# taldatech/soft-intro-vae-pytorch

Measured on AMD Instinct MI355X. Metric: training images/sec (whole node) at 256x256 bs128, higher is better.
Workload: dtype f32; 1 GPU; soft_intro_vae celeb256 256x256 zdim=512 channels=[64, 128, 256, 512, 512, 512], full E-step + D-step iteration; global_batch=128, per_gpu_batch=128, parallelism=dp1, decoder_forward_reuse=True, hip_graph=False, batchnorm=local

## Files before the change

### soft-intro-vae-pytorch_amd/csrc/conv_wino4_kernel.inc

```
template <bool PRO>
__global__ void __launch_bounds__(W4_NT, 1) W4_KERNEL_NAME(Wino4Args a) {
  constexpr int CK = W4_CK, RS = W4_RS, PLANE = W4_PLANE, XBUF = W4_XBUF, VBUF = W4_VBUF;
  __shared__ __attribute__((aligned(16))) float raw0[XBUF];
  __shared__ __attribute__((aligned(16))) float raw1[XBUF];
  __shared__ __attribute__((aligned(16))) float vx[VBUF + W4_EXF];
#define RAWB(BUF) ((BUF) ? raw1 : raw0)
  __shared__ float4 pro4[PRO ? W4_PRO_MAX : 1];

  const int tid = threadIdx.x, lane = tid & 63;
  const int wave = __builtin_amdgcn_readfirstlane(tid >> 6);
  const int l31 = lane & 31, hh = lane >> 5;
  const int wj = wave % 6, ws = wave / 6;
  const int H = a.H, W = a.W, HW = H * W;
  const int tx = l31 & 7, ty = l31 >> 3;

  const int tp = wave >> 2;
  const int ti = (wave & 3) * 64 + lane, tt = ti & 31, tc = ti >> 5;
  const int trb = tc * PLANE + 4 * (tt >> 3) * RS + 4 * (tt & 7) + 4;
  const int jA = tp == 0 ? 1 : (tp == 1 ? 3 : 0), jB = tp == 0 ? 2 : (tp == 1 ? 4 : 5);
  const int tvb = tc * 32 + tt;
  const float t_al = tp == 0 ? -4.f : -1.f;
  const float t_be = tp == 0 ? 1.f : 2.f;
  const float t_ga = tp == 0 ? -4.f : -2.f;
  const bool pair05 = tp == 2;
#if W4_GRID
  const unsigned long long seam_m0 = a.seam_c0, seam_m5 = a.seam_c5, seam_mr0 = a.seam_r0, seam_mr5 = a.seam_r5;
  const int two_w = W4_PXW, two_h = W4_PXH, two_mask = a.W - 1, two_hmask = a.H - 1, two_img = a.Ci * a.H * a.W;
  const int two_nx = W4_PXW >> a.iw_l2, two_ipi = two_nx * (W4_PXH >> a.ih_l2);
#else
  const unsigned long long seam_m0 = 0x1010101010101010ull, seam_m5 = 0x0808080808080808ull;
  const int two_w = a.two ? 32 : a.W, two_mask = a.two ? 15 : -1, two_img = a.two ? a.Ci * a.H * a.W : 0;
#endif
  const int vrb = (wj * CK + hh) * 32 + l31;

  const int dsub = wave % 3, dpl0 = wave / 3;
  const int pg = dsub * 64 + lane, prow = pg / 10, pk = pg - prow * 10;
  const bool pvalid = pg < 180;

  const int n_items = a.n_items;
  const int nchunks = a.cps;
  const int ksteps = nchunks * (CK / 2);
  const __amdgpu_buffer_rsrc_t ursrc = make_rsrc(a.up, 36ull * a.Ci_pad * a.Co_pad * 4ull);
  const unsigned va0 = (unsigned)(hh * a.Co_pad + ws * 32 + l31) * 24u;
  const unsigned ua_step = (unsigned)a.Co_pad * 24u;

  int item = blockIdx.x;
  if (a.xcd_group) item = ((int)blockIdx.x & 7) * ((int)gridDim.x >> 3) + ((int)blockIdx.x >> 3);
  int b, r0, c0, co0, pt;
  int cbase = 0, kslice = 0;
  __amdgpu_buffer_rsrc_t xrsrc;
  unsigned xo, ua_base;
  int pseg = 0;
#if W4_GRID
#define W4_SETUP_IMG                                                     \
    b = two_ipi * pt;                                                    \
    xrsrc = make_rsrc(a.x + (size_t)b * a.Ci * HW, (unsigned long long)two_ipi * a.Ci * HW * 4ull); \
    const int r = r0 - 1 + prow, c = c0 - 4 + 4 * pk;                    \
    xo = (pvalid && r >= 0 && r < two_h && c >= 0 && c < two_w)          \
             ? (unsigned)(((r >> a.ih_l2) * two_nx + (c >> a.iw_l2)) * two_img + (r & two_hmask) * W + (c & two_mask)) * 4u \
             : SIVAE_OOB;
#else
#define W4_SETUP_IMG                                                     \
    b = a.two ? 2 * pt : b;                                              \
    xrsrc = make_rsrc(a.x + (size_t)b * a.Ci * HW, (unsigned long long)(a.two ? 2 : 1) * a.Ci * HW * 4ull); \
    const int r = r0 - 1 + prow, c = c0 - 4 + 4 * pk;                    \
    xo = (pvalid && r >= 0 && r < H && c >= 0 && c < two_w)              \
             ? (unsigned)((c >> 4) * two_img + r * W + (c & two_mask)) * 4u : SIVAE_OOB;
#endif
#define W4_SETUP(ITEM)                                                   \
  {                                                                      \
    const int co_tile = (ITEM) % a.n_co_tiles;                           \
    const int iq_ = (ITEM) / a.n_co_tiles;                               \
    kslice = iq_ % a.ksl;                                                \
    pt = iq_ / a.ksl;                                                    \
    cbase = kslice * a.cps * CK;                                         \
    const int tbx = pt % a.nbw;                                          \
    const int t2 = pt / a.nbw;                                           \
    const int tby = t2 % a.nbh;                                          \
    b = t2 / a.nbh;                                                      \
    r0 = tby * W4_PXH;                                                   \
    c0 = tbx * W4_PXW;                                                   \
    co0 = co_tile * W4_TCO;                                              \
    W4_SETUP_IMG                                                         \
    ua_base = (unsigned)((wj * a.Ci_pad + cbase) * a.Co_pad + co0) * 24u; \
    if (PRO) pseg = (b / a.pro_seg_images) * a.Ci_pad + cbase;           \
  }
#define W4_DMA1(CH, BUF, N)                                              \
  if (!((W4_ABLATE & 1) && item >= 0)) {                                 \
    const int ck = dpl0 + 4 * (N);                                       \
    const int ci = cbase + (CH)*CK + ck;                                 \
    const int cic = ci < a.Ci ? ci : a.Ci - 1;                           \
    __builtin_amdgcn_raw_ptr_buffer_load_lds(                            \
        xrsrc, (float __attribute__((address_space(3)))*)(RAWB(BUF) + ck * PLANE + dsub * 256), 16, xo, \
        (unsigned)cic * (unsigned)HW * 4u, 0, 0);                        \
  }
#define W4_FIXUP(CH, BUF, XO, PSEG)                                      \
  {                                                                      \
    const float msk_ = (XO) != SIVAE_OOB ? 1.f : 0.f;                    \
    _Pragma("unroll") for (int n_ = 0; n_ < 2; ++n_) {                   \
      const int ck = dpl0 + 4 * n_;                                      \
      float4* q_ = reinterpret_cast<float4*>(RAWB(BUF) + ck * PLANE + dsub * 256 + lane * 4); \
      const float4 p_ = pro4[(PSEG) + (CH)*CK + ck];                     \
      float4 v_ = *q_;                                                   \
      v_.x = fmaf(v_.x - p_.x, p_.y, p_.z);                              \
      v_.y = fmaf(v_.y - p_.x, p_.y, p_.z);                              \
      v_.z = fmaf(v_.z - p_.x, p_.y, p_.z);                              \
      v_.w = fmaf(v_.w - p_.x, p_.y, p_.z);                              \
      v_.x = fmaxf(v_.x, v_.x * a.pro_slope) * msk_;                     \
      v_.y = fmaxf(v_.y, v_.y * a.pro_slope) * msk_;                     \
      v_.z = fmaxf(v_.z, v_.z * a.pro_slope) * msk_;                     \
      v_.w = fmaxf(v_.w, v_.w * a.pro_slope) * msk_;                     \
      *q_ = v_;                                                          \
    }                                                                    \
  }

  f32x16 acc[6];
  float4 U4[2];
  float2 U2[2];
#if W4_ABLATE & 2
  U4[0] = U4[1] = make_float4(1.f, 0.5f, 0.25f, 2.f);
  U2[0] = U2[1] = make_float2(1.f, 0.5f);
#endif
#define W4_LOAD_A(UBASE, KS_ABS, SLOT)                                   \
  if (!(W4_ABLATE & 2)) {                                                \
    const unsigned so = (UBASE) + (unsigned)(2 * (KS_ABS)) * ua_step;    \
    U4[SLOT] = buf_load_f32x4(ursrc, va0, so);                           \
    U2[SLOT] = buf_load_f32x2(ursrc, va0 + 16u, so);                     \
  }
#define W4_REFILL(CH, KK)                                                \
  {                                                                      \
    const int ks2 = (CH) * (CK / 2) + (KK) + 2;                          \
    const bool in_item = ks2 < ksteps;                                   \
    const unsigned ub_ = (in_item || !has_next) ? ua_cur : ua_base;      \
    const int kq_ = in_item ? ks2 : (has_next ? ks2 - ksteps : ksteps - 1); \
    W4_LOAD_A(ub_, kq_, (KK)&1)                                          \
  }
#define W4_FENCE __builtin_amdgcn_sched_barrier(0);
#define W4_LDS_BARRIER asm volatile("s_waitcnt lgkmcnt(0)\n\ts_barrier" ::: "memory");
#define W4_READB(VB, KK, BV)                                             \
  {                                                                      \
    const float* p_ = vx + (VB)*VBUF + 2 * (KK)*32 + vrb;                \
    _Pragma("unroll") for (int i = 0; i < 6; ++i) BV[i] = p_[i * 6 * CK * 32]; \
  }
#define W4_TREAD(RB, R0, P05)                                               \
  {                                                                      \
    const float* p_ = RAWB(RB) + trb + (R0)*RS;                          \
    _Pragma("unroll") for (int r = 0; r < 3; ++r) {                      \
      td_[r] = *reinterpret_cast<const float4*>(p_ + r * RS);            \
      if (P05) {                                                         \
        te0_[r] = p_[r * RS - 1];                                        \
        te5_[r] = p_[r * RS + 4];                                        \
        if (W4_TWO) {  \
          asm volatile("v_cndmask_b32_e64 %0, %0, 0, %1" : "+v"(te0_[r]) : "s"(seam_m0));                \
          asm volatile("v_cndmask_b32_e64 %0, %0, 0, %1" : "+v"(te5_[r]) : "s"(seam_m5));                \
// ... 62 lines not shown
     \
    if (!(W4_ABLATE & 8)) W4_LDS_BARRIER                                 \
    W4_FENCE                                                             \
                                                           \
    W4_READB(VB, 2, b0_)                                                 \
    W4_MF(0, U4[1].x, b1_) W4_MF(1, U4[1].y, b1_) W4_FENCE               \
    W4_TDOT(3, P05)                                                      \
    W4_FENCE                                                             \
    W4_MF(2, U4[1].z, b1_) W4_MF(3, U4[1].w, b1_) W4_MF(4, U2[1].x, b1_) W4_MF(5, U2[1].y, b1_) W4_FENCE \
    W4_REFILL(CH, 1)                                                     \
    W4_FENCE                                                             \
                                                           \
    W4_READB(VB, 3, b1_)                                                 \
    W4_MF(0, U4[0].x, b0_) W4_MF(1, U4[0].y, b0_) W4_MF(2, U4[0].z, b0_) W4_FENCE \
    W4_TCOL((VB) ^ 1, tA_, jA)                                           \
    W4_FENCE                                                             \
    W4_MF(3, U4[0].w, b0_) W4_MF(4, U2[0].x, b0_) W4_MF(5, U2[0].y, b0_) W4_FENCE \
    if (PRO) {                                                           \
      W4_FIXUP(FCH, VB, xo_f, pseg_f)                                    \
      W4_FENCE                                                           \
    }                                                                    \
    W4_REFILL(CH, 2)                                                     \
    W4_FENCE                                                             \
                                                           \
    W4_MF(0, U4[1].x, b1_) W4_MF(1, U4[1].y, b1_) W4_MF(2, U4[1].z, b1_) W4_FENCE \
    W4_TCOL((VB) ^ 1, tB_, jB)                                           \
    W4_FENCE                                                             \
    W4_MF(3, U4[1].w, b1_) W4_MF(4, U2[1].x, b1_) W4_MF(5, U2[1].y, b1_) W4_FENCE \
    W4_REFILL(CH, 3)                                                     \
    W4_DMA1(DCH, (VB) ^ 1, 0)                                            \
    W4_DMA1(DCH, (VB) ^ 1, 1)                                            \
    xo_f = xo;                                                           \
    pseg_f = pseg;                                                       \
    W4_FENCE                                                             \
     \
    if (!(W4_ABLATE & 8)) W4_LDS_BARRIER                                 \
  }
#define W4_TRANSFORM_ALL(RB, VN, P05)                                    \
  {                                                                      \
    float4 td_[3];                                                       \
    float te0_[3], te5_[3], tA_[6], tB_[6];                              \
    W4_TREAD(RB, 0, P05)                                                 \
    W4_TDOT(0, P05)                                                      \
    W4_TREAD(RB, 3, P05)                                                 \
    W4_TDOT(3, P05)                                                      \
    W4_TCOL(VN, tA_, jA)                                                 \
    W4_TCOL(VN, tB_, jB)                                                 \
  }
#define W4_PAIR(CH, P05)                                                 \
  {                                                                      \
    const int d0_ = (CH) + 3 < nchunks ? (CH) + 3 : (CH) + 3 - nchunks;  \
    const int f0_ = (CH) + 2 < nchunks ? (CH) + 2 : (CH) + 2 - nchunks;  \
    W4_CHUNK(CH, 0, d0_, f0_, P05)                                       \
    if ((CH) + 4 == nchunks && has_next) W4_SETUP(next)                  \
    const int d1_ = (CH) + 4 < nchunks ? (CH) + 4 : (CH) + 4 - nchunks;  \
    const int f1_ = (CH) + 3 < nchunks ? (CH) + 3 : (CH) + 3 - nchunks;  \
    W4_CHUNK((CH) + 1, 1, d1_, f1_, P05)                                 \
  }

  if (PRO) {
    for (int idx = tid; idx < a.pro_nseg * a.Ci_pad; idx += W4_NT) {
      const int c = idx % a.Ci_pad, so = (idx / a.Ci_pad) * a.Ci;
      pro4[idx] = c < a.Ci ? make_float4(a.pro_mean[so + c], a.pro_invstd[so + c] * a.pro_gamma[c], a.pro_beta[c], 0.f)
                           : make_float4(0.f, 0.f, 0.f, 0.f);
    }
    __syncthreads();
  }
  W4_SETUP(item)
  W4_DMA1(0, 0, 0)
  W4_DMA1(0, 0, 1)
  W4_DMA1(1, 1, 0)
  W4_DMA1(1, 1, 1)
  unsigned ua_cur = ua_base;
  W4_LOAD_A(ua_cur, 0, 0)
  W4_LOAD_A(ua_cur, 1, 1)
  __builtin_amdgcn_s_waitcnt(0x0F70);
  if (PRO) {
    W4_FIXUP(0, 0, xo, pseg)
    W4_FIXUP(1, 1, xo, pseg)
  }
  __syncthreads();
  if (pair05) W4_TRANSFORM_ALL(0, 0, true) else W4_TRANSFORM_ALL(0, 0, false)
  __syncthreads();
  W4_DMA1(2, 0, 0)
  W4_DMA1(2, 0, 1)
  unsigned xo_f = xo;
  int pseg_f = pseg;
#ifdef W4_TIMING
  int it_n = 0;
#endif
  for (;;) {
    W4_STAMP(0)
    W4_STAMP(6)
#pragma unroll
    for (int i = 0; i < 6; ++i)
#pragma unroll
      for (int r = 0; r < 16; ++r) acc[i][r] = 0.f;
    const int e_pt = pt, e_b = b, e_r0 = r0, e_c0 = c0, e_co0 = co0, e_ks = kslice;
    const int next = item + (int)gridDim.x;
    const bool has_next = next < n_items;
    if (pair05) {
      for (int ch = 0; ch < nchunks; ch += 2) {
        W4_PAIR(ch, true)
        W4_STAMPK(ch)
      }
    } else {
      for (int ch = 0; ch < nchunks; ch += 2) {
        W4_PAIR(ch, false)
        W4_STAMPK(ch)
      }
    }
    W4_STAMP(1)

#if W4_POOL
    {
      float* ex = vx + VBUF;
      const int Hh = H >> 1, Wh = W >> 1, HWh = Hh * Wh;
      const __amdgpu_buffer_rsrc_t yrsrc =
          make_rsrc(a.y + (size_t)e_b * a.Co * HWh, (unsigned long long)a.Co * HWh * 4ull);
      int lane_;
      asm volatile("v_mbcnt_lo_u32_b32 %0, -1, 0\n\tv_mbcnt_hi_u32_b32 %0, -1, %0" : "=v"(lane_));
// ... 174 lines not shown
```

### soft-intro-vae-pytorch_amd/csrc/conv_wino_up.hip

```cpp
#include "common.h"
#include "pack_batch.h"
#include <stdlib.h>

struct WinoUpArgs {
  const float* x;
  const float* up;
  float* y;
  const float* pro_mean;
  const float* pro_invstd;
  const float* pro_gamma;
  const float* pro_beta;
  float pro_slope;
  float* stats;
  int B, Ci, Co, H, W;
  int Ci_pad, Co_pad;
  int nbh, nbw;
  int n_co_tiles;
  int n_items;
  int xcd_group;
};

#define WUP_CK 16
#define WUP_TCO 32

// ... 28 lines not shown
  int pt, b, r0, c0, co0;
  __amdgpu_buffer_rsrc_t xrsrc;
  const __amdgpu_buffer_rsrc_t ursrc = make_rsrc(a.up, 4ull * a.Ci_pad * a.Co_pad * 48ull);
  unsigned xo, ua_base;
  static_assert(2 * NPOS >= NT, "duplicate-owner mapping");
  const int teff = tid < NPOS ? tid : tid - NPOS;
  const int xrr = teff / LWU, xcc = teff % LWU;
  const int xl = xrr * RS + (xcc & 1) * PH + (xcc >> 1);
  float xmask = 0.f;
#define WUP_SETUP(ITEM)                                                  \
  {                                                                      \
    const int co_tile = (ITEM) % a.n_co_tiles;                           \
    pt = (ITEM) / a.n_co_tiles;                                          \
    const int tbx = pt % a.nbw;                                          \
    const int t2 = pt / a.nbw;                                           \
    const int tby = t2 % a.nbh;                                          \
    b = t2 / a.nbh;                                                      \
    r0 = tby * PXH;                                                      \
    c0 = tbx * PXW;                                                      \
    co0 = co_tile * WUP_TCO;                                             \
    xrsrc = make_rsrc(a.x + (size_t)b * a.Ci * HWs, (unsigned long long)a.Ci * HWs * 4ull); \
    const int r = r0 + xrr - 1, c = c0 + xcc - 1;                        \
    xo = SIVAE_OOB;                                                      \
    xmask = 0.f;                                                         \
    if (r >= 0 && r < Hs && c >= 0 && c < Ws) {                          \
      xo = (unsigned)(r * Ws + c) * 4u;                                  \
      xmask = 1.f;                                                       \
    }                                                                    \
    ua_base = (unsigned)((wave * a.Ci_pad) * a.Co_pad + co0) * 48u;      \
  }

  const unsigned va0 = (unsigned)(hh * a.Co_pad + l31) * 48u;
  const unsigned ua_step = (unsigned)a.Co_pad * 48u;

  const int tx = l31 & (TTW - 1), ty = l31 >> TTW_L2;
  const int bb = hh * PLANE + (2 * ty + pp) * RS + tx;
  const int oc0 = ((pq + 0) & 1) * PH + ((pq + 0) >> 1);
  const int oc1 = ((pq + 1) & 1) * PH + ((pq + 1) >> 1);
  const int oc2 = ((pq + 2) & 1) * PH + ((pq + 2) >> 1);

  f32x16 acc[9];
  float xr[CK];
  float4 AR[4][3];
  const int nksteps = a.Ci_pad / 2;

#define WUP_LOAD_X(CH)                                                   \
  {                                                                      \
    _Pragma("unroll") for (int ck = 0; ck < CK; ++ck) {                  \
      const int ci = (CH)*CK + ck;                                       \
      const int cic = ci < a.Ci ? ci : a.Ci - 1;                         \
      xr[ck] = buf_load_f32(xrsrc, xo, (unsigned)cic * (unsigned)HWs * 4u); \
    }                                                                    \
  }
#define WUP_LOAD_A(KS_ABS, SLOT)                                         \
  {                                                                      \
    const unsigned so = ua_base + (unsigned)(2 * (KS_ABS)) * ua_step;    \
    AR[SLOT][0] = buf_load_f32x4(ursrc, va0, so);                        \
    AR[SLOT][1] = buf_load_f32x4(ursrc, va0 + 16u, so);                  \
    AR[SLOT][2] = buf_load_f32x4(ursrc, va0 + 32u, so);                  \
  }
#define WUP_STORE_X(CH, BUF)                                             \
  {                                                                      \
    _Pragma("unroll") for (int ck = 0; ck < CK; ++ck) {                  \
      const int ci = (CH)*CK + ck;                                       \
      float v = xr[ck];                                                  \
      if (PRO) {                                                         \
        const float4 p4 = pro4[ci];                                      \
        v = lrelu01((v - p4.x) * p4.y + p4.z, a.pro_slope) * xmask;      \
      } else {                                                           \
        v = ci < a.Ci ? v : 0.f;                                         \
      }                                                                  \
      xs[(BUF)*XBUF + ck * PLANE + xl] = v;                              \
    }                                                                    \
  }
#define WUP_READ(BUF, KK, D)                                             \
  {                                                                      \
    const float* pb_ = xs + (BUF)*XBUF + 2 * (KK)*PLANE + bb;            \
    _Pragma("unroll") for (int r = 0; r < 3; ++r) {                      \
      D[r][0] = pb_[r * RS + oc0];                                       \
      D[r][1] = pb_[r * RS + oc1];                                       \
      D[r][2] = pb_[r * RS + oc2];                                       \
    }                                                                    \
  }
#define WUP_STEP(SLOT, D)                                                \
  {                                                                      \
    float t[3][3];                                                       \
    _Pragma("unroll") for (int r = 0; r < 3; ++r) {                      \
      t[r][0] = D[r][0] - D[r][1];                                       \
      t[r][1] = D[r][1];                                                 \
      t[r][2] = D[r][1] - D[r][2];                                       \
    }                                                                    \
    _Pragma("unroll") for (int j = 0; j < 3; ++j) {                      \
      const float v0 = t[0][j] - t[1][j], v1 = t[1][j], v2 = t[1][j] - t[2][j]; \
      const float u0 = (j == 0) ? AR[SLOT][0].x : ((j == 1) ? AR[SLOT][0].y : AR[SLOT][0].z); \
      const float u1 = (j == 0) ? AR[SLOT][0].w : ((j == 1) ? AR[SLOT][1].x : AR[SLOT][1].y); \
      const float u2 = (j == 0) ? AR[SLOT][1].z : ((j == 1) ? AR[SLOT][1].w : AR[SLOT][2].x); \
      acc[0 * 3 + j] = __builtin_amdgcn_mfma_f32_32x32x2f32(u0, v0, acc[0 * 3 + j], 0, 0, 0); \
      acc[1 * 3 + j] = __builtin_amdgcn_mfma_f32_32x32x2f32(u1, v1, acc[1 * 3 + j], 0, 0, 0); \
      acc[2 * 3 + j] = __builtin_amdgcn_mfma_f32_32x32x2f32(u2, v2, acc[2 * 3 + j], 0, 0, 0); \
    }                                                                    \
  }
#define WUP_KSTEP(CH, BUF, KK, D, DN)                                    \
  {                                                                      \
    if ((KK) + 1 < CK / 2) WUP_READ(BUF, (KK) + 1, DN)                   \
    __builtin_amdgcn_sched_barrier(0);                                   \
    WUP_STEP((KK)&3, D)                                                  \
    __builtin_amdgcn_sched_barrier(0);                                   \
    if ((CH) * (CK / 2) + (KK) + 4 < nksteps) WUP_LOAD_A((CH) * (CK / 2) + (KK) + 4, (KK)&3) \
  }
#define WUP_MMA(CH, BUF, NEXT)                                           \
  {                                                                      \
    float d0[3][3], d1[3][3];                                            \
    if (NEXT) WUP_LOAD_X((CH) + 1)                                       \
    WUP_READ(BUF, 0, d0)                                                 \
    WUP_KSTEP(CH, BUF, 0, d0, d1)                                        \
    WUP_KSTEP(CH, BUF, 1, d1, d0)                                        \
    WUP_KSTEP(CH, BUF, 2, d0, d1)                                        \
    WUP_KSTEP(CH, BUF, 3, d1, d0)                                        \
    WUP_KSTEP(CH, BUF, 4, d0, d1)                                        \
    WUP_KSTEP(CH, BUF, 5, d1, d0)                                        \
    WUP_KSTEP(CH, BUF, 6, d0, d1)                                        \
    if (NEXT) WUP_STORE_X((CH) + 1, (BUF) ^ 1)                           \
    __builtin_amdgcn_sched_barrier(0);                                   \
    WUP_KSTEP(CH, BUF, 7, d1, d0)                                        \
    __syncthreads();                                                     \
  }

  const int nchunks = a.Ci_pad / CK;
  if (PRO) {
    for (int c = tid; c < a.Ci_pad; c += NT) {
      pro4[c] = c < a.Ci ? make_float4(a.pro_mean[c], a.pro_invstd[c] * a.pro_gamma[c], a.pro_beta[c], 0.f)
                         : make_float4(0.f, 0.f, 0.f, 0.f);
    }
    __syncthreads();
  }
  WUP_SETUP(item)
  WUP_LOAD_X(0)
#pragma unroll
  for (int kk = 0; kk < 4; ++kk) WUP_LOAD_A(kk, kk)
  for (;;) {
#pragma unroll
    for (int f = 0; f < 9; ++f)
#pragma unroll
      for (int r = 0; r < 16; ++r) acc[f][r] = 0.f;
    WUP_STORE_X(0, 0)
    __syncthreads();
    int ch = 0;
    for (; ch + 1 < nchunks; ch += 2) {
      WUP_MMA(ch, 0, true)
      const bool more = ch + 2 < nchunks;
      WUP_MMA(ch + 1, 1, more)
    }
    if (ch < nchunks) WUP_MMA(ch, 0, false)

    __builtin_amdgcn_s_setprio(1);
    const int e_pt = pt, e_b = b, e_r0 = r0, e_c0 = c0, e_co0 = co0;
    const int next = item + (int)gridDim.x;
    const bool has_next = next < n_items;
    if (has_next) {
      WUP_SETUP(next)
      WUP_LOAD_X(0)
#pragma unroll
      for (int kk = 0; kk < 4; ++kk) WUP_LOAD_A(kk, kk)
    }
    {
      const __amdgpu_buffer_rsrc_t yrsrc =
          make_rsrc(a.y + (size_t)e_b * a.Co * H * W, (unsigned long long)a.Co * H * W * 4ull);
      const int li = e_r0 + 2 * ty, lj = e_c0 + 2 * tx;
      const bool ok00 = li < Hs && lj < Ws, ok01 = li < Hs && lj + 1 < Ws;
      const bool ok10 = li + 1 < Hs && lj < Ws, ok11 = li + 1 < Hs && lj + 1 < Ws;
      float* exw = ex + wave * (16 * 2 * 64) + lane;
      const float* exr = ex + (wave ^ 1) * (16 * 2 * 64) + lane;
      float keep[16][2];
#pragma unroll
      for (int r = 0; r < 16; ++r) {
        const int chn = e_co0 + (r & 3) + 8 * (r >> 2) + 4 * hh;
        const float s00 = acc[0][r] + acc[3][r], s01 = acc[1][r] + acc[4][r], s02 = acc[2][r] + acc[5][r];
        const float s10 = acc[3][r] - acc[6][r], s11 = acc[4][r] - acc[7][r], s12 = acc[5][r] - acc[8][r];
        const float y00 = s00 + s01, y01 = s01 - s02, y10 = s10 + s11, y11 = s11 - s12;
        if (pq == 0) {
          keep[r][0] = y00; keep[r][1] = y01;
          exw[(r * 2 + 0) * 64] = y10; exw[(r * 2 + 1) * 64] = y11;
        } else {
          keep[r][0] = y10; keep[r][1] = y11;
          exw[(r * 2 + 0) * 64] = y00; exw[(r * 2 + 1) * 64] = y01;
        }
        if (a.stats != nullptr) {
          const bool cok = chn < a.Co;
          float s = (ok00 ? y00 : 0.f) + (ok01 ? y01 : 0.f) + (ok10 ? y10 : 0.f) + (ok11 ? y11 : 0.f);
          float q = (ok00 ? y00 * y00 : 0.f) + (ok01 ? y01 * y01 : 0.f) + (ok10 ? y10 * y10 : 0.f) +
                    (ok11 ? y11 * y11 : 0.f);
          s = half_wave_sum_hi(s);
          q = half_wave_sum_hi(q);
          if (l31 == 31 && cok) {
            float* dst = a.stats + ((size_t)(e_pt * 4 + wave) * a.Co + chn) * 2;
            dst[0] = s;
            dst[1] = q;
          }
        }
      }
      asm volatile("s_waitcnt lgkmcnt(0)\n\ts_barrier" ::: "memory");
      const bool rok = pq == 0 ? li < Hs : li + 1 < Hs;
      const unsigned base = (unsigned)((2 * (li + pq) + pp) * W + 2 * lj) * 4u;
      f32x4 f_prev = {0.f, 0.f, 0.f, 0.f};
#pragma unroll
      for (int r = 0; r < 16; ++r) {
        const int chn = e_co0 + (r & 3) + 8 * (r >> 2) + 4 * hh;
        const float o0 = exr[(r * 2 + 0) * 64], o1 = exr[(r * 2 + 1) * 64];
        const unsigned cb = base + (unsigned)chn * (unsigned)(H * W) * 4u;
        const float c0_ = pq == 0 ? keep[r][0] : o0, c1_ = pq == 0 ? o0 : keep[r][0];
        const float c2_ = pq == 0 ? keep[r][1] : o1, c3_ = pq == 0 ? o1 : keep[r][1];
        if (rok && lj < Ws && chn < a.Co) {
          typedef unsigned int u32x4_t __attribute__((ext_vector_type(4)));
          const f32x4 f = {c0_, c1_, c2_, c3_};
          __builtin_amdgcn_raw_buffer_store_b128(__builtin_bit_cast(u32x4_t, f), yrsrc, (int)cb, 0, 0);
          SIVAE_PIN4(f_prev)
          f_prev = f;
        }
      }
      SIVAE_PIN4(f_prev)
    }
    __builtin_amdgcn_s_setprio(0);
    if (!has_next) break;
    item = next;
  }
#undef WUP_SETUP
#undef WUP_LOAD_X
#undef WUP_LOAD_A
#undef WUP_STORE_X
#undef WUP_READ
#undef WUP_STEP
#undef WUP_KSTEP
#undef WUP_MMA
}

__device__ __forceinline__ void pack_wino_up_body(const float* __restrict__ w, float* __restrict__ up, int Co,
                                                           int Ci, int kpad, int npad, size_t idx0_, const size_t stride_) {
  const size_t total = (size_t)kpad * npad;
  for (size_t idx = idx0_; idx < total; idx += stride_) {
    const int n = (int)(idx % npad), k = (int)(idx / npad);
    float g[3][3];
    const bool ok = k < Ci && n < Co;
#pragma unroll
    for (int r = 0; r < 3; ++r)
#pragma unroll
      for (int c = 0; c < 3; ++c) g[r][c] = ok ? w[((size_t)n * Ci + k) * 9 + r * 3 + c] : 0.f;
#pragma unroll
    for (int p = 0; p < 2; ++p)
#pragma unroll
      for (int q = 0; q < 2; ++q) {
        float rw[2][3];
#pragma unroll
        for (int c = 0; c < 3; ++c) {
          rw[0][c] = p == 0 ? g[0][c] : g[0][c] + g[1][c];
          rw[1][c] = p == 0 ? g[1][c] + g[2][c] : g[2][c];
        }
        float gp[2][2];
#pragma unroll
        for (int a_ = 0; a_ < 2; ++a_) {
          gp[a_][0] = q == 0 ? rw[a_][0] : rw[a_][0] + rw[a_][1];
          gp[a_][1] = q == 0 ? rw[a_][1] + rw[a_][2] : rw[a_][2];
        }
        float gr[3][2];
#pragma unroll
        for (int b_ = 0; b_ < 2; ++b_) {
          gr[0][b_] = gp[0][b_];
          gr[1][b_] = gp[0][b_] + gp[1][b_];
          gr[2][b_] = gp[1][b_];
        }
        float u[12];
#pragma unroll
        for (int i = 0; i < 3; ++i) {
          u[i * 3 + 0] = gr[i][0];
          u[i * 3 + 1] = gr[i][0] + gr[i][1];
          u[i * 3 + 2] = gr[i][1];
        }
        u[9] = u[10] = u[11] = 0.f;
        float4* dst = reinterpret_cast<float4*>(up + (((size_t)(p * 2 + q) * kpad + k) * npad + n) * 12);
        dst[0] = make_float4(u[0], u[1], u[2], u[3]);
        dst[1] = make_float4(u[4], u[5], u[6], u[7]);
        dst[2] = make_float4(u[8], u[9], u[10], u[11]);
// ... 128 lines not shown
```

### soft-intro-vae-pytorch_amd/csrc/conv_wino_up_dgrad.hip

```cpp
#include "common.h"
#include "pack_batch.h"
#include <stdlib.h>

struct WinoUpDgArgs {
  const float* dyp;
  const float* ud;
  float* dx;
  int B, C, N, Hs, Ws;
  int Cpad, Npad;
  int nbh, nbw;
  int n_n_tiles;
  int n_items;
  int accumulate;
  int n_items_base;
  int q_per_split;
  long long dx_split_stride;
  int xcd_group;
};

__device__ __forceinline__ void buf_store_f32(__amdgpu_buffer_rsrc_t r, float v, unsigned voff, unsigned soff) {
  __builtin_amdgcn_raw_buffer_store_b32(__builtin_bit_cast(unsigned int, v), r, (int)voff, (int)soff, 0);
}

#define WUD_CK 16
// ... 31 lines not shown
  if (a.xcd_group) item = ((int)blockIdx.x & 7) * ((int)gridDim.x >> 3) + ((int)blockIdx.x >> 3);
  int b, r0, c0, n0;
  int q0, q1, sl;
  __amdgpu_buffer_rsrc_t xrsrc;
  const __amdgpu_buffer_rsrc_t ursrc = make_rsrc(a.ud, 4ull * a.Cpad * a.Npad * 48ull);
  unsigned xo, ua_base;
  static_assert(2 * NPOS >= 256, "duplicate-owner mapping");
  const int teff = tid < NPOS ? tid : tid - NPOS;
  const int xrr = teff / LWU, xcc = teff % LWU;
  const int xl = xrr * RS + (xcc & 1) * PH + (xcc >> 1);
#define WUD_SETUP(ITEM)                                                  \
  {                                                                      \
    sl = (ITEM) / a.n_items_base;                                        \
    const int it_ = (ITEM)-sl * a.n_items_base;                          \
    q0 = sl * a.q_per_split;                                             \
    q1 = q0 + a.q_per_split < nchunks ? q0 + a.q_per_split : nchunks;    \
    const int n_tile = it_ % a.n_n_tiles;                                \
    const int pt = it_ / a.n_n_tiles;                                    \
    const int tbx = pt % a.nbw;                                          \
    const int t2 = pt / a.nbw;                                           \
    const int tby = t2 % a.nbh;                                          \
    b = t2 / a.nbh;                                                      \
    r0 = tby * PXH;                                                      \
    c0 = tbx * PXW;                                                      \
    n0 = n_tile * (KS2 ? WUD_TN / 2 : WUD_TN);                           \
    xrsrc = make_rsrc(a.dyp + (size_t)b * 4 * a.C * HWs, 4ull * a.C * HWs * 4ull); \
    const int r = r0 + xrr - 1, c = c0 + xcc - 1;                        \
    xo = SIVAE_OOB;                                                      \
     \
    if (r >= 0 && r < Hs && c >= 0 && c < Ws) xo = (unsigned)(2 * r * (2 * Ws) + 2 * c) * 4u; \
    ua_base = (unsigned)(n0 + ng * 32) * 48u + (unsigned)koff * ua_step; \
  }

  const unsigned va0 = (unsigned)(hh * a.Npad + l31) * 48u;
  const unsigned ua_step = (unsigned)a.Npad * 48u;

  const int tx = l31 & (TTW - 1), ty = l31 >> TTW_L2;
  const int bb0 = (hh + koff) * PLANE + 2 * ty * RS + tx;
  int bc0, bc1, bc2;

  f32x16 acc[9];
  float xr[CK];
  float4 AR[4][3];

#define WUD_LOAD_X(Q)                                                    \
  {                                                                      \
    const int ph_ = (Q)&3, cc0_ = ((Q) >> 2) * CK;                           \
    _Pragma("unroll") for (int ck = 0; ck < CK; ++ck) {                  \
      const int c = cc0_ + ck;                                           \
      const int cclamp = c < a.C ? c : a.C - 1;                          \
      xr[ck] = buf_load_f32(xrsrc, xo, (unsigned)cclamp * (unsigned)HWs * 16u + (unsigned)((ph_ >> 1) * 2 * Ws + (ph_ & 1)) * 4u); \
    }                                                                    \
  }
#define WUD_LOAD_A(KS_ABS, SLOT)                                         \
  {                                                                      \
    const int q_ = (KS_ABS) / KPC;  \
    const unsigned so = ua_base + (unsigned)((q_ & 3) * a.Cpad + (q_ >> 2) * CK + 2 * ((KS_ABS) % KPC)) * ua_step; \
    AR[SLOT][0] = buf_load_f32x4(ursrc, va0, so);                        \
    AR[SLOT][1] = buf_load_f32x4(ursrc, va0 + 16u, so);                  \
    AR[SLOT][2] = buf_load_f32x4(ursrc, va0 + 32u, so);                  \
  }
#define WUD_STORE_X(Q, BUF)                                              \
  {                                                                      \
    const int ph_ = (Q)&3, cc0_ = ((Q) >> 2) * CK;                           \
    _Pragma("unroll") for (int ck = 0; ck < CK; ++ck) {                  \
      const float v = (cc0_ + ck) < a.C ? xr[ck] : 0.f;                  \
      xs[(BUF)*XBUF + ck * PLANE + xl] = v;                              \
    }                                                                    \
  }
#define WUD_BASES(Q)                                                     \
  {                                                                      \
    const int ph_ = (Q)&3;                                               \
    const int ro = 1 - (ph_ >> 1), co = 1 - (ph_ & 1);                   \
    const int base = bb0 + ro * RS;                                      \
    bc0 = base + ((co + 0) & 1) * PH + ((co + 0) >> 1);                  \
    bc1 = base + ((co + 1) & 1) * PH + ((co + 1) >> 1);                  \
    bc2 = base + ((co + 2) & 1) * PH + ((co + 2) >> 1);                  \
  }
#define WUD_READ(BUF, KK, D)                                             \
  {                                                                      \
    const float* pb_ = xs + (BUF)*XBUF + 2 * (KK)*PLANE;                 \
    _Pragma("unroll") for (int r = 0; r < 3; ++r) {                      \
      D[r][0] = pb_[r * RS + bc0];                                       \
      D[r][1] = pb_[r * RS + bc1];                                       \
      D[r][2] = pb_[r * RS + bc2];                                       \
    }                                                                    \
  }
#define WUD_STEP(SLOT, D)                                                \
  {                                                                      \
    float t[3][3];                                                       \
    _Pragma("unroll") for (int r = 0; r < 3; ++r) {                      \
      t[r][0] = D[r][0] - D[r][1];                                       \
      t[r][1] = D[r][1];                                                 \
      t[r][2] = D[r][1] - D[r][2];                                       \
    }                                                                    \
    _Pragma("unroll") for (int j = 0; j < 3; ++j) {                      \
      const float v0 = t[0][j] - t[1][j], v1 = t[1][j], v2 = t[1][j] - t[2][j]; \
      const float u0 = (j == 0) ? AR[SLOT][0].x : ((j == 1) ? AR[SLOT][0].y : AR[SLOT][0].z); \
      const float u1 = (j == 0) ? AR[SLOT][0].w : ((j == 1) ? AR[SLOT][1].x : AR[SLOT][1].y); \
      const float u2 = (j == 0) ? AR[SLOT][1].z : ((j == 1) ? AR[SLOT][1].w : AR[SLOT][2].x); \
      acc[0 * 3 + j] = __builtin_amdgcn_mfma_f32_32x32x2f32(u0, v0, acc[0 * 3 + j], 0, 0, 0); \
      acc[1 * 3 + j] = __builtin_amdgcn_mfma_f32_32x32x2f32(u1, v1, acc[1 * 3 + j], 0, 0, 0); \
      acc[2 * 3 + j] = __builtin_amdgcn_mfma_f32_32x32x2f32(u2, v2, acc[2 * 3 + j], 0, 0, 0); \
    }                                                                    \
  }
#define WUD_KSTEP(Q, BUF, KK, D, DN)                                     \
  {                                                                      \
    if ((KK) + 1 < KPC) WUD_READ(BUF, (KK) + 1, DN)                      \
    __builtin_amdgcn_sched_barrier(0);                                   \
    WUD_STEP((KK)&3, D)                                                  \
    __builtin_amdgcn_sched_barrier(0);                                   \
    if ((Q) * KPC + (KK) + 4 < q1 * KPC) WUD_LOAD_A((Q) * KPC + (KK) + 4, (KK)&3) \
  }
#define WUD_MMA(Q, BUF, NEXT)                                            \
  {                                                                      \
    float d0[3][3], d1[3][3];                                            \
    if (NEXT) WUD_LOAD_X((Q) + 1)                                        \
    WUD_BASES(Q)                                                         \
    WUD_READ(BUF, 0, d0)                                                 \
    WUD_KSTEP(Q, BUF, 0, d0, d1)                                         \
    WUD_KSTEP(Q, BUF, 1, d1, d0)                                         \
    WUD_KSTEP(Q, BUF, 2, d0, d1)                                         \
    if (!KS2) {                                                          \
      WUD_KSTEP(Q, BUF, 3, d1, d0)                                       \
      WUD_KSTEP(Q, BUF, 4, d0, d1)                                       \
      WUD_KSTEP(Q, BUF, 5, d1, d0)                                       \
      WUD_KSTEP(Q, BUF, 6, d0, d1)                                       \
    }                                                                    \
    if (NEXT) WUD_STORE_X((Q) + 1, (BUF) ^ 1)                            \
    __builtin_amdgcn_sched_barrier(0);                                   \
    if (KS2) WUD_KSTEP(Q, BUF, 3, d1, d0) else WUD_KSTEP(Q, BUF, 7, d1, d0) \
    __syncthreads();                                                     \
  }
#define WUD_PREFETCH(ITEM)                                               \
  {                                                                      \
    WUD_SETUP(ITEM)                                                      \
    WUD_LOAD_X(q0)                                                       \
    _Pragma("unroll") for (int kk = 0; kk < 4; ++kk) WUD_LOAD_A(q0 * KPC + kk, kk) \
  }

  WUD_PREFETCH(item)
  for (;;) {
#pragma unroll
    for (int f = 0; f < 9; ++f)
#pragma unroll
      for (int r = 0; r < 16; ++r) acc[f][r] = 0.f;
    WUD_STORE_X(q0, 0)
    __syncthreads();
    int q = q0;
    for (; q + 1 < q1; q += 2) {
      WUD_MMA(q, 0, true)
      const bool more = q + 2 < q1;
      WUD_MMA(q + 1, 1, more)
    }
    if (q < q1) WUD_MMA(q, 0, false)

    __builtin_amdgcn_s_setprio(1);
    const int e_b = b, e_r0 = r0, e_c0 = c0, e_n0 = n0, e_sl = sl;
    const int next = item + (int)gridDim.x;
    const bool has_next = next < n_items;
    const bool early = has_next && !a.accumulate;
    if (early) WUD_PREFETCH(next)
    {
      const __amdgpu_buffer_rsrc_t yrsrc =
          make_rsrc(a.dx + (size_t)e_sl * a.dx_split_stride + (size_t)e_b * a.N * HWs, (unsigned long long)a.N * HWs * 4ull);
      const int li = e_r0 + 2 * ty, lj = e_c0 + 2 * tx;
      const bool okc = lj < Ws;
      const unsigned base = (unsigned)(li * Ws + lj) * 4u;
      float* red = smem;
#pragma unroll
      for (int r = 0; r < 16; ++r) {
        const float s00 = acc[0][r] + acc[3][r], s01 = acc[1][r] + acc[4][r], s02 = acc[2][r] + acc[5][r];
        const float s10 = acc[3][r] - acc[6][r], s11 = acc[4][r] - acc[7][r], s12 = acc[5][r] - acc[8][r];
        acc[0][r] = s00 + s01;
        acc[1][r] = s01 - s02;
        acc[2][r] = s10 + s11;
        acc[3][r] = s11 - s12;
      }
      if (KS2) {
        if (kh == 1) {
#pragma unroll
          for (int r = 0; r < 16; ++r)
#pragma unroll
            for (int k = 0; k < 4; ++k) red[((ng * 64) + r * 4 + k) * 64 + lane] = acc[k][r];
        }
        __syncthreads();
        if (kh == 0) {
#pragma unroll
          for (int r = 0; r < 16; ++r)
#pragma unroll
            for (int k = 0; k < 4; ++k) acc[k][r] += red[((ng * 64) + r * 4 + k) * 64 + lane];
        }
      }
      if (!KS2 || kh == 0) {
#pragma unroll
        for (int r = 0; r < 16; ++r) {
          const int chn = e_n0 + ng * 32 + (r & 3) + 8 * (r >> 2) + 4 * hh;
          float y00 = acc[0][r], y01 = acc[1][r], y10 = acc[2][r], y11 = acc[3][r];
          const bool cok = chn < a.N && okc;
          const unsigned cb = base + (unsigned)chn * (unsigned)HWs * 4u;
          const unsigned o0 = (cok && li < Hs) ? cb : SIVAE_OOB;
          const unsigned o1 = (cok && li + 1 < Hs) ? cb + (unsigned)Ws * 4u : SIVAE_OOB;
          if (AL8) {
            if (a.accumulate) {
              const float2 p0 = buf_load_f32x2(yrsrc, o0, 0u), p1 = buf_load_f32x2(yrsrc, o1, 0u);
              y00 += p0.x;
              y01 += p0.y;
              y10 += p1.x;
              y11 += p1.y;
            }
            buf_store_f32x2(yrsrc, y00, y01, o0, 0u);
            buf_store_f32x2(yrsrc, y10, y11, o1, 0u);
          } else {
            const unsigned o0b = o0 == SIVAE_OOB ? SIVAE_OOB : o0 + 4u, o1b = o1 == SIVAE_OOB ? SIVAE_OOB : o1 + 4u;
            if (a.accumulate) {
              y00 += buf_load_f32(yrsrc, o0, 0u);
              y01 += buf_load_f32(yrsrc, o0b, 0u);
              y10 += buf_load_f32(yrsrc, o1, 0u);
              y11 += buf_load_f32(yrsrc, o1b, 0u);
            }
            buf_store_f32(yrsrc, y00, o0, 0u);
            buf_store_f32(yrsrc, y01, o0b, 0u);
            buf_store_f32(yrsrc, y10, o1, 0u);
            buf_store_f32(yrsrc, y11, o1b, 0u);
          }
        }
      }
      if (KS2) __syncthreads();
    }
    if (has_next && !early) WUD_PREFETCH(next)
    __builtin_amdgcn_s_setprio(0);
    if (!has_next) break;
    item = next;
  }
#undef WUD_SETUP
#undef WUD_LOAD_X
#undef WUD_LOAD_A
#undef WUD_STORE_X
#undef WUD_BASES
#undef WUD_READ
#undef WUD_STEP
#undef WUD_KSTEP
#undef WUD_MMA
#undef WUD_PREFETCH
}

__global__ void __launch_bounds__(256) space_to_depth2_kernel(const float* __restrict__ in, float* __restrict__ out,
                                                              int C, int Hs, int Ws, size_t n_pairs) {
  const size_t stride = (size_t)gridDim.x * 256;
  const int W2 = Ws >> 1, W = 2 * Ws;
  for (size_t o = (size_t)blockIdx.x * 256 + threadIdx.x; o < n_pairs; o += stride) {
    const int j2 = (int)(o % W2);
    size_t t = o / W2;
    const int i = (int)(t % Hs);
    t /= Hs;
    const int c = (int)(t % C);
    const size_t bb = t / C;
    const float* src = in + ((t * 2 * Hs + 2 * i) * (size_t)W) + 4 * j2;
    const float4 r0 = *reinterpret_cast<const float4*>(src);
    const float4 r1 = *reinterpret_cast<const float4*>(src + W);
    const size_t plane = (size_t)Hs * Ws;
    float* dst = out + ((bb * 4 * C + c) * Hs + i) * (size_t)Ws + 2 * j2;
    *reinterpret_cast<float2*>(dst) = make_float2(r0.x, r0.z);
    *reinterpret_cast<float2*>(dst + (size_t)C * plane) = make_float2(r0.y, r0.w);
    *reinterpret_cast<float2*>(dst + (size_t)2 * C * plane) = make_float2(r1.x, r1.z);
    *reinterpret_cast<float2*>(dst + (size_t)3 * C * plane) = make_float2(r1.y, r1.w);
  }
}

extern "C" int sivae_space_to_depth2(const float* in, float* out, int B, int C, int Hs, int Ws, hipStream_t stream) {
  if (!in || !out) return SIVAE_ERR_NULL;
  if (B <= 0 || C <= 0 || Hs <= 0 || Ws <= 0 || (Ws & 1)) return SIVAE_ERR_SHAPE;
  const size_t n_pairs = (size_t)B * C * Hs * (Ws >> 1);
  int nb = cdiv((long long)n_pairs, 256 * 2);
  if (nb > 8192) nb = 8192;
  if (nb < 1) nb = 1;
  hipLaunchKernelGGL(space_to_depth2_kernel, dim3(nb), dim3(256), 0, stream, in, out, C, Hs, Ws, n_pairs);
  return sivae_launch_status();
}

__device__ __forceinline__ void pack_wino_up_dgrad_body(const float* __restrict__ w, float* __restrict__ ud,
                                                                 int Co, int Ci, int cpad, int npad, size_t idx0_, const size_t stride_) {
  const size_t total = (size_t)cpad * npad;
  for (size_t idx = idx0_; idx < total; idx += stride_) {
    const int n = (int)(idx % npad), k = (int)(idx / npad);
    float g[3][3];
    const bool ok = k < Co && n < Ci;
#pragma unroll
    for (int r = 0; r < 3; ++r)
#pragma unroll
// ... 223 lines not shown
```

Measured before the change: 341.8 img/s.

## Prefetch next work item's inputs and weights during the tail of the MMA loop

In the persistent Winograd upsample forward and dgrad kernels, the next item's setup, X load and weight-register refills now happen inside the final MMA chunk instead of after the loop, so loads overlap the remaining compute and the epilogue. Lane indices are recomputed via mbcnt in the epilogue and fixup paths, presumably to reduce register pressure from keeping lane-derived values live. The dgrad path drops the accumulate-dependent early/late prefetch split, so loads of the next item's data are issued before the epilogue's read-modify-write even when accumulating. This adds address logic and register pressure and risks ordering hazards in the wrap-around indexing.

```diff
diff --git a/soft-intro-vae-pytorch_amd/csrc/conv_wino4_kernel.inc b/soft-intro-vae-pytorch_amd/csrc/conv_wino4_kernel.inc
--- a/soft-intro-vae-pytorch_amd/csrc/conv_wino4_kernel.inc
+++ b/soft-intro-vae-pytorch_amd/csrc/conv_wino4_kernel.inc
@@ -55,20 +55,30 @@
 #define W4_SETUP_IMG                                                     \
     b = two_ipi * pt;                                                    \
     xrsrc = make_rsrc(a.x + (size_t)b * a.Ci * HW, (unsigned long long)two_ipi * a.Ci * HW * 4ull); \
-    const int r = r0 - 1 + prow, c = c0 - 4 + 4 * pk;                    \
-    xo = (pvalid && r >= 0 && r < two_h && c >= 0 && c < two_w)          \
+    const int r = r0 - 1 + prow_, c = c0 - 4 + 4 * pk_;                  \
+    xo = (pvalid_ && r >= 0 && r < two_h && c >= 0 && c < two_w)         \
              ? (unsigned)(((r >> a.ih_l2) * two_nx + (c >> a.iw_l2)) * two_img + (r & two_hmask) * W + (c & two_mask)) * 4u \
              : SIVAE_OOB;
 #else
 #define W4_SETUP_IMG                                                     \
     b = a.two ? 2 * pt : b;                                              \
     xrsrc = make_rsrc(a.x + (size_t)b * a.Ci * HW, (unsigned long long)(a.two ? 2 : 1) * a.Ci * HW * 4ull); \
-    const int r = r0 - 1 + prow, c = c0 - 4 + 4 * pk;                    \
-    xo = (pvalid && r >= 0 && r < H && c >= 0 && c < two_w)              \
+    const int r = r0 - 1 + prow_, c = c0 - 4 + 4 * pk_;                  \
+    xo = (pvalid_ && r >= 0 && r < H && c >= 0 && c < two_w)             \
              ? (unsigned)((c >> 4) * two_img + r * W + (c & two_mask)) * 4u : SIVAE_OOB;
 #endif
-#define W4_SETUP(ITEM)                                                   \
-  {                                                                      \
+#define W4_SETUP(ITEM, INLOOP)                                           \
+  {                                                                      \
+    int prow_ = prow, pk_ = pk;                                          \
+    bool pvalid_ = pvalid;                                               \
+    if (PRO && (INLOOP)) {                                               \
+      int l_;                                                            \
+      asm volatile("v_mbcnt_lo_u32_b32 %0, -1, 0\n\tv_mbcnt_hi_u32_b32 %0, -1, %0" : "=v"(l_)); \
+      const int pg_ = dsub * 64 + l_;                                    \
+      prow_ = pg_ / 10;                                                  \
+      pk_ = pg_ - prow_ * 10;                                            \
+      pvalid_ = pg_ < 180;                                               \
+    }                                                                    \
     const int co_tile = (ITEM) % a.n_co_tiles;                           \
     const int iq_ = (ITEM) / a.n_co_tiles;                               \
     kslice = iq_ % a.ksl;                                                \
@@ -97,9 +107,11 @@
 #define W4_FIXUP(CH, BUF, XO, PSEG)                                      \
   {                                                                      \
     const float msk_ = (XO) != SIVAE_OOB ? 1.f : 0.f;                    \
+    int fl_ = lane;                                                      \
+    if (W4_GRID) asm volatile("v_mbcnt_lo_u32_b32 %0, -1, 0\n\tv_mbcnt_hi_u32_b32 %0, -1, %0" : "=v"(fl_)); \
     _Pragma("unroll") for (int n_ = 0; n_ < 2; ++n_) {                   \
       const int ck = dpl0 + 4 * n_;                                      \
-      float4* q_ = reinterpret_cast<float4*>(RAWB(BUF) + ck * PLANE + dsub * 256 + lane * 4); \
+      float4* q_ = reinterpret_cast<float4*>(RAWB(BUF) + ck * PLANE + dsub * 256 + fl_ * 4); \
       const float4 p_ = pro4[(PSEG) + (CH)*CK + ck];                     \
       float4 v_ = *q_;                                                   \
       v_.x = fmaf(v_.x - p_.x, p_.y, p_.z);                              \
@@ -268,7 +280,7 @@
     const int d0_ = (CH) + 3 < nchunks ? (CH) + 3 : (CH) + 3 - nchunks;  \
     const int f0_ = (CH) + 2 < nchunks ? (CH) + 2 : (CH) + 2 - nchunks;  \
     W4_CHUNK(CH, 0, d0_, f0_, P05)                                       \
-    if ((CH) + 4 == nchunks && has_next) W4_SETUP(next)                  \
+    if ((CH) + 4 == nchunks && has_next) W4_SETUP(next, true)            \
     const int d1_ = (CH) + 4 < nchunks ? (CH) + 4 : (CH) + 4 - nchunks;  \
     const int f1_ = (CH) + 3 < nchunks ? (CH) + 3 : (CH) + 3 - nchunks;  \
     W4_CHUNK((CH) + 1, 1, d1_, f1_, P05)                                 \
@@ -282,7 +294,7 @@
     }
     __syncthreads();
   }
-  W4_SETUP(item)
+  W4_SETUP(item, false)
   W4_DMA1(0, 0, 0)
   W4_DMA1(0, 0, 1)
   W4_DMA1(1, 1, 0)
diff --git a/soft-intro-vae-pytorch_amd/csrc/conv_wino_up.hip b/soft-intro-vae-pytorch_amd/csrc/conv_wino_up.hip
--- a/soft-intro-vae-pytorch_amd/csrc/conv_wino_up.hip
+++ b/soft-intro-vae-pytorch_amd/csrc/conv_wino_up.hip
@@ -104,12 +104,20 @@
       xr[ck] = buf_load_f32(xrsrc, xo, (unsigned)cic * (unsigned)HWs * 4u); \
     }                                                                    \
   }
-#define WUP_LOAD_A(KS_ABS, SLOT)                                         \
-  {                                                                      \
-    const unsigned so = ua_base + (unsigned)(2 * (KS_ABS)) * ua_step;    \
+#define WUP_LOAD_A(UBASE, KS_ABS, SLOT)                                  \
+  {                                                                      \
+    const unsigned so = (UBASE) + (unsigned)(2 * (KS_ABS)) * ua_step;    \
     AR[SLOT][0] = buf_load_f32x4(ursrc, va0, so);                        \
     AR[SLOT][1] = buf_load_f32x4(ursrc, va0 + 16u, so);                  \
     AR[SLOT][2] = buf_load_f32x4(ursrc, va0 + 32u, so);                  \
+  }
+#define WUP_REFILL(CH, KK)                                               \
+  {                                                                      \
+    const int ks4 = (CH) * (CK / 2) + (KK) + 4;                          \
+    const bool in_item = ks4 < nksteps;                                  \
+    const unsigned ub_ = (in_item || !has_next) ? ua_cur : ua_base;      \
+    const int kq_ = in_item ? ks4 : (has_next ? ks4 - nksteps : nksteps - 1); \
+    WUP_LOAD_A(ub_, kq_, (KK)&3)                                         \
   }
 #define WUP_STORE_X(CH, BUF)                                             \
   {                                                                      \
@@ -158,12 +166,15 @@
     __builtin_amdgcn_sched_barrier(0);                                   \
     WUP_STEP((KK)&3, D)                                                  \
     __builtin_amdgcn_sched_barrier(0);                                   \
-    if ((CH) * (CK / 2) + (KK) + 4 < nksteps) WUP_LOAD_A((CH) * (CK / 2) + (KK) + 4, (KK)&3) \
-  }
-#define WUP_MMA(CH, BUF, NEXT)                                           \
+    WUP_REFILL(CH, KK)                                                   \
+  }
+#define WUP_MMA(CH, BUF, MAYEND)                                         \
   {                                                                      \
     float d0[3][3], d1[3][3];                                            \
-    if (NEXT) WUP_LOAD_X((CH) + 1)                                       \
+    const bool more_ = !(MAYEND) || (CH) + 1 < nchunks;                  \
+    if ((MAYEND) && !more_ && has_next) WUP_SETUP(next)                  \
+    const int xc_ = more_ ? (CH) + 1 : (has_next ? 0 : (CH));            \
+    WUP_LOAD_X(xc_)                                                      \
     WUP_READ(BUF, 0, d0)                                                 \
     WUP_KSTEP(CH, BUF, 0, d0, d1)                                        \
     WUP_KSTEP(CH, BUF, 1, d1, d0)                                        \
@@ -172,7 +183,7 @@
     WUP_KSTEP(CH, BUF, 4, d0, d1)                                        \
     WUP_KSTEP(CH, BUF, 5, d1, d0)                                        \
     WUP_KSTEP(CH, BUF, 6, d0, d1)                                        \
-    if (NEXT) WUP_STORE_X((CH) + 1, (BUF) ^ 1)                           \
+    if (more_) WUP_STORE_X((CH) + 1, (BUF) ^ 1)                          \
     __builtin_amdgcn_sched_barrier(0);                                   \
     WUP_KSTEP(CH, BUF, 7, d1, d0)                                        \
     __syncthreads();                                                     \
@@ -189,32 +200,26 @@
   WUP_SETUP(item)
   WUP_LOAD_X(0)
 #pragma unroll
-  for (int kk = 0; kk < 4; ++kk) WUP_LOAD_A(kk, kk)
+  for (int kk = 0; kk < 4; ++kk) WUP_LOAD_A(ua_base, kk, kk)
   for (;;) {
 #pragma unroll
     for (int f = 0; f < 9; ++f)
 #pragma unroll
       for (int r = 0; r < 16; ++r) acc[f][r] = 0.f;
+    const int e_pt = pt, e_b = b, e_r0 = r0, e_c0 = c0, e_co0 = co0;
+    const unsigned ua_cur = ua_base;
+    const int next = item + (int)gridDim.x;
+    const bool has_next = next < n_items;
     WUP_STORE_X(0, 0)
     __syncthreads();
     int ch = 0;
     for (; ch + 1 < nchunks; ch += 2) {
-      WUP_MMA(ch, 0, true)
-      const bool more = ch + 2 < nchunks;
-      WUP_MMA(ch + 1, 1, more)
+      WUP_MMA(ch, 0, false)
+      WUP_MMA(ch + 1, 1, true)
     }
-    if (ch < nchunks) WUP_MMA(ch, 0, false)
+    if (ch < nchunks) WUP_MMA(ch, 0, true)
 
     __builtin_amdgcn_s_setprio(1);
-    const int e_pt = pt, e_b = b, e_r0 = r0, e_c0 = c0, e_co0 = co0;
-    const int next = item + (int)gridDim.x;
-    const bool has_next = next < n_items;
-    if (has_next) {
-      WUP_SETUP(next)
-      WUP_LOAD_X(0)
-#pragma unroll
-      for (int kk = 0; kk < 4; ++kk) WUP_LOAD_A(kk, kk)
-    }
     {
       const __amdgpu_buffer_rsrc_t yrsrc =
           make_rsrc(a.y + (size_t)e_b * a.Co * H * W, (unsigned long long)a.Co * H * W * 4ull);
@@ -279,6 +284,7 @@
 #undef WUP_SETUP
 #undef WUP_LOAD_X
 #undef WUP_LOAD_A
+#undef WUP_REFILL
 #undef WUP_STORE_X
 #undef WUP_READ
 #undef WUP_STEP
diff --git a/soft-intro-vae-pytorch_amd/csrc/conv_wino_up_dgrad.hip b/soft-intro-vae-pytorch_amd/csrc/conv_wino_up_dgrad.hip
--- a/soft-intro-vae-pytorch_amd/csrc/conv_wino_up_dgrad.hip
+++ b/soft-intro-vae-pytorch_amd/csrc/conv_wino_up_dgrad.hip
@@ -107,13 +107,21 @@
       xr[ck] = buf_load_f32(xrsrc, xo, (unsigned)cclamp * (unsigned)HWs * 16u + (unsigned)((ph_ >> 1) * 2 * Ws + (ph_ & 1)) * 4u); \
     }                                                                    \
   }
-#define WUD_LOAD_A(KS_ABS, SLOT)                                         \
+#define WUD_LOAD_A(UBASE, KS_ABS, SLOT)                                  \
   {                                                                      \
     const int q_ = (KS_ABS) / KPC;  \
-    const unsigned so = ua_base + (unsigned)((q_ & 3) * a.Cpad + (q_ >> 2) * CK + 2 * ((KS_ABS) % KPC)) * ua_step; \
+    const unsigned so = (UBASE) + (unsigned)((q_ & 3) * a.Cpad + (q_ >> 2) * CK + 2 * ((KS_ABS) % KPC)) * ua_step; \
     AR[SLOT][0] = buf_load_f32x4(ursrc, va0, so);                        \
     AR[SLOT][1] = buf_load_f32x4(ursrc, va0 + 16u, so);                  \
     AR[SLOT][2] = buf_load_f32x4(ursrc, va0 + 32u, so);                  \
+  }
+#define WUD_REFILL(Q, KK)                                                \
+  {                                                                      \
+    const int ks4 = (Q) * KPC + (KK) + 4;                                \
+    const bool in_item = ks4 < e_q1 * KPC;                               \
+    const unsigned ub_ = (in_item || !has_next) ? ua_cur : ua_base;      \
+    const int kq_ = in_item ? ks4 : (has_next ? q0 * KPC + (ks4 - e_q1 * KPC) : e_q1 * KPC - 1); \
+    WUD_LOAD_A(ub_, kq_, (KK)&3)                                         \
   }
 #define WUD_STORE_X(Q, BUF)                                              \
   {                                                                      \
@@ -165,12 +173,15 @@
     __builtin_amdgcn_sched_barrier(0);                                   \
     WUD_STEP((KK)&3, D)                                                  \
     __builtin_amdgcn_sched_barrier(0);                                   \
-    if ((Q) * KPC + (KK) + 4 < q1 * KPC) WUD_LOAD_A((Q) * KPC + (KK) + 4, (KK)&3) \
-  }
-#define WUD_MMA(Q, BUF, NEXT)                                            \
+    WUD_REFILL(Q, KK)                                                    \
+  }
+#define WUD_MMA(Q, BUF, MAYEND)                                          \
   {                                                                      \
     float d0[3][3], d1[3][3];                                            \
-    if (NEXT) WUD_LOAD_X((Q) + 1)                                        \
+    const bool more_ = !(MAYEND) || (Q) + 1 < e_q1;                      \
+    if ((MAYEND) && !more_ && has_next) WUD_SETUP(next)                  \
+    const int xq_ = more_ ? (Q) + 1 : (has_next ? q0 : (Q));             \
+    WUD_LOAD_X(xq_)                                                      \
     WUD_BASES(Q)                                                         \
     WUD_READ(BUF, 0, d0)                                                 \
     WUD_KSTEP(Q, BUF, 0, d0, d1)                                         \
@@ -182,7 +193,7 @@
       WUD_KSTEP(Q, BUF, 5, d1, d0)                                       \
       WUD_KSTEP(Q, BUF, 6, d0, d1)                                       \
     }                                                                    \
-    if (NEXT) WUD_STORE_X((Q) + 1, (BUF) ^ 1)                            \
+    if (more_) WUD_STORE_X((Q) + 1, (BUF) ^ 1)                           \
     __builtin_amdgcn_sched_barrier(0);                                   \
     if (KS2) WUD_KSTEP(Q, BUF, 3, d1, d0) else WUD_KSTEP(Q, BUF, 7, d1, d0) \
     __syncthreads();                                                     \
@@ -191,7 +202,7 @@
   {                                                                      \
     WUD_SETUP(ITEM)                                                      \
     WUD_LOAD_X(q0)                                                       \
-    _Pragma("unroll") for (int kk = 0; kk < 4; ++kk) WUD_LOAD_A(q0 * KPC + kk, kk) \
+    _Pragma("unroll") for (int kk = 0; kk < 4; ++kk) WUD_LOAD_A(ua_base, q0 * KPC + kk, kk) \
   }
 
   WUD_PREFETCH(item)
@@ -200,26 +211,27 @@
     for (int f = 0; f < 9; ++f)
 #pragma unroll
       for (int r = 0; r < 16; ++r) acc[f][r] = 0.f;
-    WUD_STORE_X(q0, 0)
-    __syncthreads();
-    int q = q0;
-    for (; q + 1 < q1; q += 2) {
-      WUD_MMA(q, 0, true)
-      const bool more = q + 2 < q1;
-      WUD_MMA(q + 1, 1, more)
-    }
-    if (q < q1) WUD_MMA(q, 0, false)
-
-    __builtin_amdgcn_s_setprio(1);
-    const int e_b = b, e_r0 = r0, e_c0 = c0, e_n0 = n0, e_sl = sl;
+    const int e_b = b, e_r0 = r0, e_c0 = c0, e_n0 = n0, e_sl = sl, e_q0 = q0, e_q1 = q1;
+    const unsigned ua_cur = ua_base;
     const int next = item + (int)gridDim.x;
     const bool has_next = next < n_items;
-    const bool early = has_next && !a.accumulate;
-    if (early) WUD_PREFETCH(next)
+    WUD_STORE_X(e_q0, 0)
+    __syncthreads();
+    int q = e_q0;
+    for (; q + 1 < e_q1; q += 2) {
+      WUD_MMA(q, 0, false)
+      WUD_MMA(q + 1, 1, true)
+    }
+    if (q < e_q1) WUD_MMA(q, 0, true)
+
+    __builtin_amdgcn_s_setprio(1);
     {
       const __amdgpu_buffer_rsrc_t yrsrc =
           make_rsrc(a.dx + (size_t)e_sl * a.dx_split_stride + (size_t)e_b * a.N * HWs, (unsigned long long)a.N * HWs * 4ull);
-      const int li = e_r0 + 2 * ty, lj = e_c0 + 2 * tx;
+      int lane_;
+      asm volatile("v_mbcnt_lo_u32_b32 %0, -1, 0\n\tv_mbcnt_hi_u32_b32 %0, -1, %0" : "=v"(lane_));
+      const int hh_ = lane_ >> 5, tx_ = lane_ & (TTW - 1), ty_ = (lane_ & 31) >> TTW_L2;
+      const int li = e_r0 + 2 * ty_, lj = e_c0 + 2 * tx_;
       const bool okc = lj < Ws;
       const unsigned base = (unsigned)(li * Ws + lj) * 4u;
       float* red = smem;
@@ -237,20 +249,20 @@
 #pragma unroll
           for (int r = 0; r < 16; ++r)
 #pragma unroll
-            for (int k = 0; k < 4; ++k) red[((ng * 64) + r * 4 + k) * 64 + lane] = acc[k][r];
+            for (int k = 0; k < 4; ++k) red[((ng * 64) + r * 4 + k) * 64 + lane_] = acc[k][r];
         }
         __syncthreads();
         if (kh == 0) {
 #pragma unroll
           for (int r = 0; r < 16; ++r)
 #pragma unroll
-            for (int k = 0; k < 4; ++k) acc[k][r] += red[((ng * 64) + r * 4 + k) * 64 + lane];
+            for (int k = 0; k < 4; ++k) acc[k][r] += red[((ng * 64) + r * 4 + k) * 64 + lane_];
         }
       }
       if (!KS2 || kh == 0) {
 #pragma unroll
         for (int r = 0; r < 16; ++r) {
-          const int chn = e_n0 + ng * 32 + (r & 3) + 8 * (r >> 2) + 4 * hh;
+          const int chn = e_n0 + ng * 32 + (r & 3) + 8 * (r >> 2) + 4 * hh_;
           float y00 = acc[0][r], y01 = acc[1][r], y10 = acc[2][r], y11 = acc[3][r];
           const bool cok = chn < a.N && okc;
           const unsigned cb = base + (unsigned)chn * (unsigned)HWs * 4u;
@@ -283,7 +295,6 @@
       }
       if (KS2) __syncthreads();
     }
-    if (has_next && !early) WUD_PREFETCH(next)
     __builtin_amdgcn_s_setprio(0);
     if (!has_next) break;
     item = next;
@@ -291,6 +302,7 @@
 #undef WUD_SETUP
 #undef WUD_LOAD_X
 #undef WUD_LOAD_A
+#undef WUD_REFILL
 #undef WUD_STORE_X
 #undef WUD_BASES
 #undef WUD_READ
```

Measured after the change: 342.5 img/s (median of 3 runs). Within noise of the previous version (+0.2%).
